# garg02/mpi-sppy

Hardware: AMD Instinct MI355X
Metric: PH scenario-iterations/sec (farmer 100k) + time to conv<1e-4 (higher is better)
Workload: dtype f64; 1 GPU; farmer crops_multiplier=1, 100000 scenarios (BASELINE configs[2]); scenarios=100000, scenarios_per_gpu=100000, n=12, m=7, nonants=3, parallelism=scenario-sharded x1, RCCL allreduce

## Files before the change

mpi-sppy_amd/csrc/phx_jit.h:

```cpp
#pragma once
#include <stdint.h>
#include <math.h>
#include <stdio.h>
#include <algorithm>
#include <sstream>
#include <string>
#include <vector>
#include "phx_setup.h"

namespace phx {

struct LaneStructure {
    int n = 0, m = 0, nnz = 0, npairs = 0, nvar = 0, nslot = 0;
    bool c_vary = false, bnd_vary = false, rhs_vary = false;
    bool scaled = false;
    std::vector<int32_t> row, col, kvar, col_slot;
    std::vector<int32_t> pair_a, pair_b, pair_pos;
    std::vector<uint8_t> lnz;
    std::vector<uint8_t> rfirst, cfirst, rempty, cempty;
    std::vector<uint8_t> lfin, ufin, fixed, blfin, bufin, eq;
    std::vector<double> Ac, dc, dr, c, lb, ub, bl, bu;
    double ipm_xs = 1.0, ipm_zs = 1.0, ipm_ws = 1.0;
    double multi_theta = 0.0;
    int multi_rounds = 0;
// ... 137 lines not shown
    o << "}; return a[k]; }\n";
}

inline void emit_dtable(std::ostringstream& o, const char* name, const std::vector<double>& v) {
    o << "  __host__ __device__ static constexpr double " << name << "(int k) { constexpr double a[] = {";
    char buf[64];
    for (size_t i = 0; i < v.size(); ++i) {
        snprintf(buf, sizeof(buf), "%a", std::isfinite(v[i]) ? v[i] : 0.0);
        o << (i ? "," : "") << buf;
    }
    if (v.empty()) o << "0.0";
    o << "}; return a[k]; }\n";
}

enum LaneKernel {
    LK_COLD, LK_COLD_AS, LK_WARM, LK_WARM_LIST, LK_MAP, LK_TAIL, LK_SEED, LK_WARM_FZ1, LK_WARM_FZR2, LK_ALL,
    LK_LIST_ALL, LK_ALL_RL, LK_ALL_PK, LK_COUNT
};
constexpr const char* LANE_KERNEL_NAMES[] = {
    "phx_lane_cold", "phx_lane_cold_as", "phx_lane_warm", "phx_lane_warm_list", "phx_lane_map", "phx_fz_tail",
    "phx_lane_seed", "phx_lane_warm_fz1", "phx_lane_warm_fzr2", "phx_lane_all", "phx_lane_list_all",
    "phx_lane_all_rl", "phx_lane_all_pk"};
static_assert(sizeof(LANE_KERNEL_NAMES) / sizeof(LANE_KERNEL_NAMES[0]) == LK_COUNT, "one name per LaneKernel");

inline std::string lane_kernel_source(const LaneStructure& L, int warm_waves = 1, bool with_map = false,
                                      int cold_waves = 1) {
    const std::string wl = with_map ? "phx_lane::warm_lane<PT, true>" : "phx_lane::warm_lane<PT, false>";
    std::ostringstream o;
    o << "#include \"phx_lane.h\"\n";
    o << "struct PT {\n";
    o << "  static constexpr int NMAX_N = " << L.n << ", NMAX_M = " << L.m << ", NMAX_K = " << L.nnz
      << ", NMAX_V = " << std::max(L.nvar, 1) << ", NMAX_S = " << std::max(L.nslot, 1) << ";\n";
    o << "  __host__ __device__ static constexpr int nvar() { return " << L.nvar << "; }\n";
    o << "  __host__ __device__ static constexpr bool scaled() { return " << (L.scaled ? "true" : "false") << "; }\n";
    o << "  __host__ __device__ static constexpr int nslot() { return " << L.nslot << "; }\n";
    o << "  __host__ __device__ static constexpr int n() { return " << L.n << "; }\n";
    o << "  __host__ __device__ static constexpr int m() { return " << L.m << "; }\n";
    o << "  __host__ __device__ static constexpr int nnz() { return " << L.nnz << "; }\n";
    o << "  __host__ __device__ static constexpr int npairs() { return " << L.npairs << "; }\n";
    o << "  __host__ __device__ static constexpr bool c_vary() { return " << (L.c_vary ? "true" : "false") << "; }\n";
    o << "  __host__ __device__ static constexpr bool bnd_vary() { return " << (L.bnd_vary ? "true" : "false")
      << "; }\n";
    o << "  __host__ __device__ static constexpr bool rhs_vary() { return " << (L.rhs_vary ? "true" : "false")
      << "; }\n";
    {
        char buf[512];
// ... 50 lines not shown
    emit_dtable(o, "bls", L.bl);
    emit_dtable(o, "bus", L.bu);
    o << "};\n";
    o << "extern \"C\" __global__ void __launch_bounds__(64, " << warm_waves
      << ") phx_lane_warm(phx_lane::LaneIO io) {\n"
         "  phx_lane::lane_stamp(io, 0);\n"
         "  if (phx_lane::gated(io.gate)) return;\n"
         "  phx_lane::zero_next_counts(io.counts_next);\n"
         "  phx_lane::lane_stamp(io, 1);\n"
         "  const int t = blockIdx.x * 64 + threadIdx.x;\n"
         "  bool still = false;\n"
         "  if (t < io.S) {\n"
         "    phx_lane::lane_stamp(io, 2);\n"
         "    still = " + wl + "(io, t);\n"
         "  }\n"
         "  phx_lane::lane_stamp(io, 3);\n"
         "  phx_lane::compact_lane(still, t, io.lanes_out, io.count_out);\n"
         "  phx_lane::lane_stamp(io, 4);\n"
         "  phx_lane::lane_stamp(io, 5);\n"
         "}\n";
    o << "extern \"C\" __global__ void __launch_bounds__(64, 1) phx_lane_warm_fz1(phx_lane::LaneIO io) {\n"
         "  phx_lane::warm_fused<PT>(io);\n"
         "}\n";
    o << "extern \"C\" __global__ void __launch_bounds__(64, 2) phx_lane_warm_fzr2(phx_lane::LaneIO io) {\n"
         "  phx_lane::warm_fused<PT, PHX_FZR2_CARRY_DEF, PHX_FZR2_PARK_DEF>(io);\n"
         "}\n";
    o << "extern \"C\" __global__ void __launch_bounds__(64, 1) phx_lane_all(phx_lane::LaneIO io, int rescue) {\n"
         "  if (phx_lane::gated(io.gate)) return;\n"
         "  phx_lane::zero_next_counts(io.counts_next);\n"
         "  const int t = blockIdx.x * 64 + threadIdx.x;\n"
         "  bool still = false;\n"
         "  if (t < io.S) still = phx_lane::all_lane<PT>(io, t, rescue);\n"
         "  phx_lane::compact_lane(still, t, io.lanes_out, io.count_out);\n"
         "}\n";
    o << "extern \"C\" __global__ void __launch_bounds__(64, 1) phx_lane_all_rl(phx_lane::LaneIO io, int rescue) {\n"
         "  if (phx_lane::gated(io.gate)) return;\n"
         "  phx_lane::zero_next_counts(io.counts_next);\n"
         "  const int t = blockIdx.x * 64 + threadIdx.x;\n"
         "  bool still = false;\n"
         "  if (t < io.S) still = phx_lane::all_lane<PT, false>(io, t, rescue);\n"
         "  phx_lane::compact_lane(still, t, io.lanes_out, io.count_out);\n"
         "}\n";
    o << "extern \"C\" __global__ void __launch_bounds__(64, 1) phx_lane_all_pk(phx_lane::LaneIO io, int rescue) {\n"
         "  __shared__ double pk[phx_lane::Data<PT>::PARK * 64];\n"
         "  if (phx_lane::gated(io.gate)) return;\n"
         "  phx_lane::zero_next_counts(io.counts_next);\n"
         "  const int t = blockIdx.x * 64 + threadIdx.x;\n"
         "  bool still = false;\n"
         "  if (t < io.S) still = phx_lane::all_lane<PT, false, true>(io, t, rescue, pk);\n"
         "  phx_lane::compact_lane(still, t, io.lanes_out, io.count_out);\n"
         "}\n";
    o << "extern \"C\" __global__ void __launch_bounds__(64) phx_fz_tail(phx_lane::LaneIO io, phx_lane::TailCopy tc) {\n"
         "  phx_lane::tail_copy(tc);\n"
         "  if (phx_lane::gated(io.gate)) return;\n"
         "  (void)phx_lane::fz_decide(io.fz, io.fz.iter);\n"
         "}\n";
    o << "extern \"C\" __global__ void __launch_bounds__(64, 4) phx_lane_map(phx_lane::LaneIO io) {\n"
         "  if (phx_lane::gated(io.gate)) return;\n"
         "  phx_lane::zero_next_counts(io.counts_next);\n"
         "  const int t = blockIdx.x * 64 + threadIdx.x;\n"
         "  bool still = false;\n"
         "  if (t < io.S) still = phx_lane::map_lane<PT>(io, t);\n"
         "  phx_lane::compact_lane(still, t, io.lanes_out, io.count_out);\n"
         "}\n";
    const std::string wlr = with_map ? "phx_lane::warm_lane<PT, true, true>" : "phx_lane::warm_lane<PT, false, true>";
    o << "#ifdef PHX_LIST_RELOAD\n#define PHX_LIST_WAVES " << warm_waves << "\n#define PHX_LIST_FN " << wl
      << "\n#else\n#define PHX_LIST_WAVES 1\n#define PHX_LIST_FN " << wlr << "\n#endif\n";
    o << "extern \"C\" __global__ void __launch_bounds__(64, PHX_LIST_WAVES"
      << ") phx_lane_warm_list(phx_lane::LaneIO io, const int* lanes, const int* count) {\n"
         "  if (phx_lane::gated(io.gate)) return;\n"
         "  const int nl = *count;\n"
         "  for (int base = blockIdx.x * 64; base < nl; base += gridDim.x * 64) {\n"
         "    const int t = base + threadIdx.x;\n"
// ... 55 lines not shown
```

mpi-sppy_amd/csrc/phx_kernels.hip:

```cpp
#include <hip/hip_runtime.h>
#include <stdio.h>
#include <string.h>
#include <math.h>
#include <string>
#include <vector>
#include <algorithm>
#include "../../include/phx.h"
#include "phx_core.h"
#include "phx_setup.h"
#include "phx_wg.h"
#include "phx_sp.h"
#include "phx_jit.h"
#include "phx_lane.h"
#include <hip/hiprtc.h>
#include <rccl/rccl.h>
#include <map>
#include <memory>
#include <mutex>
#include <stdlib.h>
#include <atomic>
#include <chrono>

#include "phx_lane_src.inc"

// ... 1698 lines not shown
    double* lane_zero_d = nullptr;
    int32_t* lane_zero_i = nullptr;
    double* lane_ipm_x = nullptr;
    double* lane_ipm_y = nullptr;
    hipFunction_t lane_warm_fn = nullptr;
    hipFunction_t lane_warm_list_fn = nullptr;
    hipFunction_t lane_map_fn = nullptr;
    hipFunction_t lane_tail_fn = nullptr;
    hipFunction_t lane_seed_fn = nullptr;
    hipFunction_t lane_warm_fz1_fn = nullptr;
    hipFunction_t lane_warm_fzr2_fn = nullptr;
    hipFunction_t lane_all_fn = nullptr;
    hipFunction_t lane_list_all_fn = nullptr;
    uint32_t* aset = nullptr;
    double* lane_map = nullptr;
    uint64_t* lane_stamps = nullptr;
    const double *lane_Av = nullptr, *lane_lb = nullptr, *lane_ub = nullptr, *lane_bl = nullptr,
                 *lane_bu = nullptr;
    bool have_aset = false;
    bool aset_fresh = false;
    std::unique_ptr<LaneStructure> lane_L;
    int lane_ww = 2, lane_cw = 1;
    std::string lane_defs;
    LaneMod mod_ph, mod_fix;
    bool fix_built = false;
    bool fix_ok = false;
    bool fix_lane = false;
    double *fix_lb = nullptr, *fix_ub = nullptr;
    bool ovr_base_ok = false;
    const double* fix_vals = nullptr;
    const int32_t* fix_idx = nullptr;
    int32_t* donor_dev = nullptr;
    int donor_cap = 0;
    std::vector<int32_t> donor_lo, donor_hi;
    const void* donor_key[3] = {nullptr, nullptr, nullptr};
    int donor_key_n[2] = {0, 0};
    const double *ph_W = nullptr, *ph_rho = nullptr, *ph_xbar = nullptr;
    const int32_t* ph_idx = nullptr;
    int32_t ph_W_on = 0, ph_prox_on = 0;
    bool ph_dirty = false;
    int32_t* counts = nullptr;
    unsigned int* tickets = nullptr;
    int32_t* lane_counts = nullptr;
    int lane_parity = 0;
    std::string jit_info = "off: not built";
    int32_t* flags_dummy = nullptr;
// ... 570 lines not shown
            const char* mapenv = getenv("PHX_LANE_MAP");
            const bool want_map = mw <= 512 && mapenv && atoi(mapenv) == 1;
            const char* cw = getenv("PHX_COLD_WAVES");
            std::string src = lane_kernel_source(L, ww ? std::max(1, atoi(ww)) : 2, want_map,
                                                 cw ? std::max(1, atoi(cw)) : 1);
            if (const char* defs = getenv("PHX_LANE_DEFS")) {
                std::string pre, tok;
                for (const char* p = defs;; ++p) {
                    if (*p == ' ' || *p == 0) {
                        const size_t eq = tok.find('=');
                        if (eq != std::string::npos) tok[eq] = ' ';
                        if (!tok.empty()) pre += "#define " + tok + "\n";
                        tok.clear();
                        if (*p == 0) break;
                    } else {
                        tok += *p;
                    }
                }
                src = pre + src;
                ctx->lane_defs = pre;
            }
            ctx->lane_ww = ww ? std::max(1, atoi(ww)) : 2;
            ctx->lane_cw = cw ? std::max(1, atoi(cw)) : 1;
            if (const char* dump = getenv("PHX_LANE_SRC_DUMP")) {
                if (FILE* f = fopen(dump, "w")) {
                    fputs(src.c_str(), f);
                    fclose(f);
                }
            }
            LaneFns fns{};
            const std::string err = jit_compile(src, &fns);
            if (!err.empty()) fns = LaneFns{};
            ctx->lane_cold_fn = fns.fn[phx::LK_COLD];
            ctx->lane_cold_as_fn = fns.fn[phx::LK_COLD_AS];
            ctx->lane_warm_fn = fns.fn[phx::LK_WARM];
            ctx->lane_warm_list_fn = fns.fn[phx::LK_WARM_LIST];
            ctx->lane_map_fn = fns.fn[phx::LK_MAP];
            ctx->lane_tail_fn = fns.fn[phx::LK_TAIL];
            ctx->lane_seed_fn = fns.fn[phx::LK_SEED];
            ctx->lane_warm_fz1_fn = fns.fn[phx::LK_WARM_FZ1];
            ctx->lane_warm_fzr2_fn = fns.fn[phx::LK_WARM_FZR2];
            ctx->lane_list_all_fn = fns.fn[phx::LK_LIST_ALL];
            ctx->lane_all_fn = fns.fn[phx::LK_ALL];
            bool all_rl = false, all_pk = false;
            if (err.empty()) {
                int scratch = 0;
// ... 14 lines not shown
            if (err.empty()) {
                ctx->lane_L.reset(new LaneStructure(L));
                const size_t nw = (size_t)phx_lane::aset_words(n, m) * S;
                ctx->aset = ctx->alloc<uint32_t>(nw);
                ctx->lane_ipm_x = ctx->alloc<double>((size_t)n * S);
                ctx->lane_ipm_y = ctx->alloc<double>((size_t)std::max(m, 1) * S);
                PHX_REQUIRE(ctx, ctx->lane_ipm_x != nullptr && ctx->lane_ipm_y != nullptr,
                            "phx_set_problem: out of device memory (ipm point)");
                {
                    const size_t NS = (size_t)std::max(ctx->N, 1) * S;
                    ctx->lane_zero_d = ctx->alloc<double>(NS);
                    ctx->lane_zero_i = ctx->alloc<int32_t>(NS);
                    PHX_REQUIRE(ctx, ctx->lane_zero_d != nullptr && ctx->lane_zero_i != nullptr,
                                "phx_set_problem: out of device memory (lane stand-ins)");
                    PHX_CHECK(ctx, hipMemset(ctx->lane_zero_d, 0, sizeof(double) * NS));
                    PHX_CHECK(ctx, hipMemset(ctx->lane_zero_i, 0, sizeof(int32_t) * NS));
                }
                ctx->seed_buf = ctx->alloc<int32_t>(2 * SEED_T + 2);
                ctx->seed_aset = ctx->alloc<uint32_t>((size_t)SEED_T * phx_lane::aset_words(n, m));
                PHX_REQUIRE(ctx, ctx->aset != nullptr && ctx->seed_buf != nullptr,
                            "phx_set_problem: out of device memory (aset)");
                PHX_CHECK(ctx, hipMemset(ctx->aset, 0, sizeof(uint32_t) * nw));
                if (getenv("PHX_LANE_STAMPS") && atoi(getenv("PHX_LANE_STAMPS")) == 1) {
                    const size_t ns = (size_t)nblk(S, PHX_BLOCK) * 8;
                    ctx->lane_stamps = ctx->alloc<uint64_t>(ns);
                    if (ctx->lane_stamps) PHX_CHECK(ctx, hipMemset(ctx->lane_stamps, 0, sizeof(uint64_t) * ns));
                }
                if (want_map) {
                    ctx->lane_map = ctx->alloc<double>(mw * S);
                    PHX_REQUIRE(ctx, ctx->lane_map != nullptr, "phx_set_problem: out of device memory (map)");
                }
            }
        } else {
            ctx->jit_info = "off: " + why;
        }
    }
    hipLaunchKernelGGL(k_norm_init, dim3(nblk(S, PHX_BLOCK)), dim3(PHX_BLOCK), 0, 0, St, S);
    if (launch_begin(ctx, 0, 0, nullptr)) return 1;
    PHX_CHECK(ctx, hipGetLastError());
    PHX_CHECK(ctx, hipDeviceSynchronize());
    if (ctx->wg_ok && !ctx->lane_cold_fn && getenv("PHX_WG_NO_FACTOR_CACHE") == nullptr) {
        const int64_t stride = (int64_t)m * (m | 1) + m;
        const int64_t kst = ((int64_t)n + m + 7) / 8 * 8;
        if ((double)S * (double)(stride * 8 + kst + 8 * (N + 1) + 4) <= 4e9) {
            ctx->wg.fac = ctx->alloc<double>((size_t)S * stride);
            ctx->wg.key = ctx->alloc<int8_t>((size_t)S * kst);
            ctx->wg.pkey = ctx->alloc<double>((size_t)S * (N + 1));
// ... 617 lines not shown
        lmax = std::max(lmax, (double)(s[5] - s[0]));
        ++nw;
    }
    if (!nw) return;
    {
        double lt[9] = {0}, sv[9] = {0}, lmx[9] = {0};
        int cnt[9] = {0};
        for (unsigned b = 0; b < G; ++b) {
            const uint64_t* s = h.data() + (size_t)b * 8;
            if (!s[0] || !s[5] || s[5] < s[0]) continue;
            const int r = (int)std::min<uint64_t>(s[6], 8);
            lt[r] += (double)(s[5] - s[0]);
            sv[r] += (double)(s[3] - s[2]);
            lmx[r] = std::max(lmx[r], (double)(s[5] - s[0]));
            ++cnt[r];
        }
        fprintf(stderr, "[lane stamps] by most rounds in the wave:");
        for (int r = 0; r <= 8; ++r)
            if (cnt[r])
                fprintf(stderr, " %d: %d waves, life %.2f (max %.2f) solve %.2f us;", r, cnt[r], lt[r] / cnt[r] * 0.01,
                        lmx[r] * 0.01, sv[r] / cnt[r] * 0.01);
        fprintf(stderr, "\n");
    }
    fprintf(stderr,
            "[lane stamps] waves %d span %.2f us, last start +%.2f us, first end +%.2f us; per wave lifetime "
            "%.2f us (max %.2f): prologue %.2f, update_w %.2f, solve %.2f, compact %.2f, epilogue %.2f us\n",
            nw, (tend - t0) * 0.01, (last_start - t0) * 0.01, (first_end - t0) * 0.01, life / nw * 0.01, lmax * 0.01,
            ph[0] / nw * 0.01, ph[1] / nw * 0.01, ph[2] / nw * 0.01, ph[3] / nw * 0.01, ph[4] / nw * 0.01);
    (void)hipMemset(ctx->lane_stamps, 0, sizeof(uint64_t) * h.size());
}

static int rescue_rounds(const phx_solve_opts* o) {
    return o->rescue_rounds > 0 ? o->rescue_rounds : std::max(16, 8 * std::max(1, o->as_rounds));
}

static int launch_cold(phx_ctx* ctx, phx_lane::LaneIO& io, const int32_t* lanes, const int32_t* count, unsigned grid,
                       hipStream_t st) {
    void* cargs[] = {&io, &lanes, &count};
    PHX_CHECK(ctx, hipModuleLaunchKernel(ctx->lane_cold_fn, grid, 1, 1, PHX_BLOCK, 1, 1, 0, st, cargs, nullptr));
    PHX_CHECK(ctx, hipModuleLaunchKernel(ctx->lane_cold_as_fn, grid, 1, 1, PHX_BLOCK, 1, 1, 0, st, cargs, nullptr));
    return 0;
}

static int enqueue_seeded_solve(phx_ctx* ctx, const phx_solve_opts* o, hipStream_t st, int32_t* C, double* x_out,
                                double* y_out, double* obj_out, int32_t* status_out, int32_t* iters_out,
                                int* npass_out) {
// ... 22 lines not shown
    }
    int32_t* next = ctx->lane_counts + 16 * ctx->lane_parity;
    io.warm_rounds = o->as_rounds;
    io.single_after = 1;
    io.lanes_out = ctx->lanesA;
    io.count_out = C;
    io.counts_next = next;
    {
        void* wargs[] = {&io};
        PHX_CHECK(ctx, hipModuleLaunchKernel(ctx->lane_warm_fn, G, 1, 1, PHX_BLOCK, 1, 1, 0, st, wargs, nullptr));
    }
    PHX_CHECK(ctx, hipGetLastError());
    io.counts_next = nullptr;
    io.lanes_out = ctx->lanesB;
    io.count_out = C + 1;
    io.as_rounds = std::max(io.as_rounds, rescue_rounds(o));
    const int32_t* in_l = ctx->lanesA;
    const int32_t* in_c = C;
    if (launch_cold(ctx, io, in_l, in_c, Gl, st)) return 1;
    *npass_out = 1;
    return 0;
}

static hipFunction_t fused_kernel(const phx_ctx* ctx, unsigned G) {
    static const bool fzr2_off = getenv("PHX_FZR2") && atoi(getenv("PHX_FZR2")) == 0;
    return (!fzr2_off && (int64_t)G > (int64_t)ctx->simds) ? ctx->lane_warm_fzr2_fn : ctx->lane_warm_fz1_fn;
}

static int enqueue_lane_solve(phx_ctx* ctx, const phx_solve_opts* o, hipStream_t st, int32_t* C, double* x_out,
                              double* y_out, double* obj_out, int32_t* status_out, int32_t* iters_out,
                              const int32_t* gate, hipEvent_t ev_a, hipEvent_t ev_b, hipEvent_t ev_c,
                              int* npass_out, unsigned cold_blocks = 0,
                              const phx_lane::FusedW* fz = nullptr, int mode = 0) {
    const int S = ctx->S;
    const unsigned G = nblk(S, PHX_BLOCK);
    phx_lane::LaneIO io = lane_io(ctx, o, x_out, y_out, obj_out, status_out, iters_out, gate);
    io.fz = fz ? *fz : phx_lane::FusedW{};
    if (fz) io.xbar_node = fz->stage;
    const bool warm_as = ctx->have_aset && o->as_rounds > 0 && ctx->lane_warm_fn;
    const bool use_map = ctx->lane_map != nullptr && ctx->lane_map_fn != nullptr;
    int npass = warm_as ? (use_map ? 2 : std::max(1, std::min(o->warm_passes, 8))) : 0;
    int32_t* next = ctx->lane_counts + 16 * ctx->lane_parity;
    int32_t* L[2] = {ctx->lanesA, ctx->lanesB};
    static const bool no_all = getenv("PHX_NO_ALL") && atoi(getenv("PHX_NO_ALL")) == 1;
    if (mode == 0 && !fz && warm_as && !use_map && npass == 1 && ctx->lane_all_fn && !no_all &&
        (int64_t)G <= (int64_t)ctx->simds) {
        if (ev_a) PHX_CHECK(ctx, ev_record(ctx, ev_a, st));
        io.lanes_out = L[0]; io.count_out = C;
        io.counts_next = next;
        io.warm_rounds = o->as_rounds;
        int resc = rescue_rounds(o);
        void* aargs[] = {&io, &resc};
        PHX_CHECK(ctx, hipModuleLaunchKernel(ctx->lane_all_fn, G, 1, 1, PHX_BLOCK, 1, 1, 0, st, aargs, nullptr));
        if (ev_b) PHX_CHECK(ctx, ev_record(ctx, ev_b, st));
        *npass_out = 0;
        return 0;
    }
    const unsigned Gl = std::min<unsigned>(G, 1024u);
    const unsigned Gc = cold_blocks ? std::min<unsigned>(G, cold_blocks) : Gl;
    if (ev_a) PHX_CHECK(ctx, ev_record(ctx, ev_a, st));
    for (int k = 0; k < npass && mode != 2; ++k) {
        io.lanes_out = L[k & 1]; io.count_out = C + k;
        io.counts_next = k == 0 ? next : nullptr;
        io.warm_rounds = use_map ? (k == 0 ? 0 : o->as_rounds) : (npass > 1 ? 1 : o->as_rounds);
        if (k == 0) {
            void* wargs[] = {&io};
            hipFunction_t fn = use_map ? ctx->lane_map_fn : (fz ? fused_kernel(ctx, G) : ctx->lane_warm_fn);
            PHX_CHECK(ctx, hipModuleLaunchKernel(fn, G, 1, 1, PHX_BLOCK, 1, 1, 0, st, wargs, nullptr));
            if (ev_b) PHX_CHECK(ctx, ev_record(ctx, ev_b, st));
        } else {
            const int32_t* in_l = L[(k - 1) & 1];
            const int32_t* in_c = C + k - 1;
            void* largs[] = {&io, &in_l, &in_c};
            PHX_CHECK(ctx, hipModuleLaunchKernel(ctx->lane_warm_list_fn, Gl, 1, 1, PHX_BLOCK, 1, 1, 0, st,
                                                 largs, nullptr));
        }
    }
    if (npass == 0 && ev_b) PHX_CHECK(ctx, ev_record(ctx, ev_b, st));
    *npass_out = npass;
    if (mode == 1) return 0;

    io.fz = phx_lane::FusedW{};
    if (mode == 2) io.xbar_node = ctx->ph_xbar;
    if (warm_as && !use_map) {
        const int32_t* in_l = L[(npass - 1) & 1];
        const int32_t* in_c = C + npass - 1;
        io.lanes_out = L[npass & 1]; io.count_out = C + npass;
        io.counts_next = nullptr;
        io.warm_rounds = rescue_rounds(o);
        io.single_after = 1;
        static const bool list_all_off = getenv("PHX_LIST_ALL") && atoi(getenv("PHX_LIST_ALL")) == 0;
// ... 1307 lines not shown
```

mpi-sppy_amd/csrc/phx_lane.h:

```cpp
#pragma once
#if !defined(__HIPCC_RTC__)
#include <stdint.h>
#include <math.h>
#if defined(__HIPCC__)
#include <hip/hip_runtime.h>
#endif
#else
typedef long long int64_t;
typedef int int32_t;
typedef unsigned int uint32_t;
typedef unsigned long long uint64_t;
#endif

#if defined(__HIPCC__) || defined(__HIPCC_RTC__)
#define PHX_LD __host__ __device__ __forceinline__
#define PHX_UNROLL _Pragma("unroll")
#define PHX_NOUNROLL _Pragma("nounroll")
#else
#define PHX_LD inline
#define PHX_UNROLL
#define PHX_NOUNROLL
#endif
#ifdef PHX_IPM_PASS_ROLLED
#define PHX_IPM_PASS_LOOP PHX_NOUNROLL
// ... 116 lines not shown
    double kkt_tol;
    double reg;
    int32_t refine;
    int32_t as_rounds;
    int32_t warm_rounds;
    int32_t single_after;
    const int32_t* gate;
    double* map;
    FusedW fz;
    uint64_t* stamps;
};

struct TailCopy {
    int32_t* left_dst;
    const int32_t* left_src;
    double* seg_dst;
    const double* seg_src;
    int32_t nseg;
    double* exp_dst;
    const double* exp_src;
};

#if defined(__HIPCC__) || defined(__HIPCC_RTC__)
__device__ __forceinline__ void lane_stamp(const LaneIO& io, int k) {
    if (io.stamps && threadIdx.x == 0) io.stamps[(uint64_t)blockIdx.x * 8 + k] = wall_clock64();
}
#endif

#if (defined(__HIPCC__) || defined(__HIPCC_RTC__)) && !defined(PHX_OUT_PLAIN)
#define PHX_OUT(lv, v) __hip_atomic_store(&(lv), (v), __ATOMIC_RELAXED, __HIP_MEMORY_SCOPE_AGENT)
#else
#define PHX_OUT(lv, v) ((lv) = (v))
#endif

PHX_LD bool gated(const int32_t* gate) { return gate && *(const volatile int32_t*)gate; }

PHX_LD void opaque(double& v) {
#if defined(__HIP_DEVICE_COMPILE__) || defined(__HIPCC_RTC__)
    __asm__ volatile("" : "+v"(v));
#else
    (void)v;
#endif
}
PHX_LD int opaque_index(int v) {
#if defined(__HIP_DEVICE_COMPILE__) || defined(__HIPCC_RTC__)
    __asm__ volatile("" : "+v"(v));
#endif
    return v;
// ... 36 lines not shown
            const double xb = io.xbar_node[fzon ? t : xi[t]];
            const double r = pon ? rv[t] : 0.0;
            const double w = won ? wv[t] : 0.0;
            qn[t] = w - r * xb;
            pn[t] = r;
            kn += 0.5 * r * xb * xb;
        }
    }
    PHX_LD Data(const LaneIO& io_, int sc_, const double* av_, const double* wv, const double* rv, const double* xbv)
        : io(io_), sc(sc_) {
        PHX_UNROLL for (int v = 0; v < PT::nvar(); ++v) av[v] = av_[v];
        const bool won = io.W_on != 0, pon = io.prox_on != 0;
        kn = 0.0;
        PHX_UNROLL for (int t = 0; t < PT::nslot(); ++t) {
            const double xb = xbv[t];
            const double r = pon ? rv[t] : 0.0;
            const double w = won ? wv[t] : 0.0;
            qn[t] = w - r * xb;
            pn[t] = r;
            kn += 0.5 * r * xb * xb;
        }
    }
    static constexpr int PARK = PT::NMAX_V + 2 * PT::NMAX_S + 1;
    PHX_LD Data(const LaneIO& io_, int sc_, const double* lds, int lane) : io(io_), sc(sc_) {
        const int l = opaque_index(lane);
        PHX_UNROLL for (int v = 0; v < PT::nvar(); ++v) av[v] = lds[v * 64 + l];
        PHX_UNROLL for (int t = 0; t < PT::nslot(); ++t) {
            qn[t] = lds[(PT::NMAX_V + t) * 64 + l];
            pn[t] = lds[(PT::NMAX_V + PT::NMAX_S + t) * 64 + l];
        }
        kn = lds[(PT::NMAX_V + 2 * PT::NMAX_S) * 64 + l];
    }
    PHX_LD void park(double* lds, int lane) const {
        PHX_UNROLL for (int v = 0; v < PT::nvar(); ++v) lds[v * 64 + lane] = av[v];
        PHX_UNROLL for (int t = 0; t < PT::nslot(); ++t) {
            lds[(PT::NMAX_V + t) * 64 + lane] = qn[t];
            lds[(PT::NMAX_V + PT::NMAX_S + t) * 64 + lane] = pn[t];
        }
        lds[(PT::NMAX_V + 2 * PT::NMAX_S) * 64 + lane] = kn;
    }
    PHX_LD double A(int k) const { return PT::kvar(k) < 0 ? PT::Ac(k) : av[PT::kvar(k)]; }
    PHX_LD double dc(int j) const { return PT::scaled() ? PT::dcs(j) : 1.0; }
    PHX_LD double dr(int i) const { return PT::scaled() ? PT::drs(i) : 1.0; }
    PHX_LD double idc(int j) const { return PT::scaled() ? PT::idcs(j) : 1.0; }
    PHX_LD double idr(int i) const { return PT::scaled() ? PT::idrs(i) : 1.0; }
    PHX_LD double c(int j) const { return PT::c_vary() ? io.c[(int64_t)j * io.S + sc] : PT::cs(j); }
    PHX_LD double q(int j) const {
        return PT::col_slot(j) >= 0 ? c(j) + dc(j) * qn[PT::col_slot(j)] : c(j);
    }
    PHX_LD double p(int j) const {
        return PT::col_slot(j) >= 0 ? dc(j) * dc(j) * pn[PT::col_slot(j)] : 0.0;
    }
    PHX_LD double l(int j) const { return PT::bnd_vary() ? io.lb[(int64_t)j * io.S + sc] : PT::lbs(j); }
    PHX_LD double u(int j) const { return PT::bnd_vary() ? io.ub[(int64_t)j * io.S + sc] : PT::ubs(j); }
    PHX_LD double bl(int i) const { return PT::rhs_vary() ? io.bl[(int64_t)i * io.S + sc] : PT::bls(i); }
    PHX_LD double bu(int i) const { return PT::rhs_vary() ? io.bu[(int64_t)i * io.S + sc] : PT::bus(i); }

    PHX_LD void matvec(const double* xv, double* ax) const {
        PHX_UNROLL for (int i = 0; i < PT::m(); ++i) if (PT::rempty(i)) ax[i] = 0.0;
        PHX_UNROLL for (int k = 0; k < PT::nnz(); ++k) {
            const double v = A(k) * xv[PT::col(k)];
            ax[PT::row(k)] = PT::rfirst(k) ? v : ax[PT::row(k)] + v;
// ... 1444 lines not shown
}

__device__ bool fz_prologue(const LaneIO& io) {
    const FusedW& f = io.fz;
    if (!f.first && fz_decide(f, f.iter - 1)) return false;
    if (f.stage[2 * f.nns] > 0.5) {
        if (blockIdx.x == 0 && threadIdx.x == 0) {
            f.ctl[1] = f.iter;
            *(volatile int32_t*)f.ctl = 2;
            publish_progress(f.prog, f.iter, 2, 0.0);
        }
        return false;
    }
    if (blockIdx.x == 0)
        for (int e = threadIdx.x; e < 2 * f.nns; e += blockDim.x) f.node_sums[e] = f.stage[e];
    return true;
}

template <class PT>
__device__ void fz_fold(const LaneIO& io, double* v) {
    const FusedW& f = io.fz;
    constexpr int NS = PT::nslot() > 0 ? PT::nslot() : 1;
    constexpr int NV = 2 * NS + 1;
    PHX_UNROLL for (int e = 0; e < NV; ++e) v[e] = wave_sum(v[e]);
    const unsigned nb = gridDim.x, b = blockIdx.x, k = b % TICKET_SHARDS;
    const unsigned nk = (nb - k + TICKET_SHARDS - 1) / TICKET_SHARDS;
    const unsigned nsh = nb < TICKET_SHARDS ? nb : TICKET_SHARDS;
    double* shard_part = f.part + (int64_t)nb * NV;
    __shared__ unsigned s_state;
    if (threadIdx.x == 0) {
        PHX_UNROLL for (int e = 0; e < NV; ++e) store_wt(&f.part[(int64_t)b * NV + e], v[e]);
        asm volatile("s_waitcnt vmcnt(0)" ::: "memory");
        PHX_HANDOFF_RELEASE();
        s_state = __hip_atomic_fetch_add(f.tk + k * TICKET_STRIDE, 1u, __ATOMIC_RELAXED,
                                         __HIP_MEMORY_SCOPE_AGENT) == nk - 1u;
    }
    __syncthreads();
    if (!s_state) return;
    PHX_HANDOFF_ACQUIRE();
    PHX_UNROLL for (int e = 0; e < NV; ++e) v[e] = 0.0;
    for (unsigned i0 = threadIdx.x; i0 < nk; i0 += 4 * 64) {
        double l[4][NV];
        PHX_UNROLL for (int u = 0; u < 4; ++u) {
            const unsigned i = i0 + 64u * u;
            PHX_UNROLL for (int e = 0; e < NV; ++e)
                l[u][e] = i < nk ? load_wt(&f.part[(int64_t)(k + TICKET_SHARDS * i) * NV + e]) : 0.0;
        }
        PHX_UNROLL for (int u = 0; u < 4; ++u) PHX_UNROLL for (int e = 0; e < NV; ++e) v[e] += l[u][e];
    }
    PHX_UNROLL for (int e = 0; e < NV; ++e) v[e] = wave_sum(v[e]);
    __syncthreads();
    if (threadIdx.x == 0) {
        PHX_UNROLL for (int e = 0; e < NV; ++e) store_wt(&shard_part[k * NV + e], v[e]);
        asm volatile("s_waitcnt vmcnt(0)" ::: "memory");
        PHX_HANDOFF_RELEASE();
        const bool last = __hip_atomic_fetch_add(f.tk + TICKET_SHARDS * TICKET_STRIDE, 1u, __ATOMIC_RELAXED,
                                                 __HIP_MEMORY_SCOPE_AGENT) == nsh - 1u;
        if (last)
            for (int q = 0; q <= TICKET_SHARDS; ++q) f.tk[q * TICKET_STRIDE] = 0u;
        s_state = last ? 2u : 0u;
    }
    __syncthreads();
    if (s_state != 2u) return;
    PHX_HANDOFF_ACQUIRE();
    const int e = threadIdx.x;
    if (e < NV) {
        double a = 0.0;
        for (unsigned q = 0; q < nsh; ++q) a += load_wt(&shard_part[q * NV + e]);
        if (e < NS) f.stage[e] = a;
        else if (e < 2 * NS) f.stage[f.nns + (e - NS)] = a;
        else {
            for (int r = 0; r < f.R; ++r) f.stage[2 * f.nns + 1 + r] = r == f.g ? a : 0.0;
            f.stage[2 * f.nns] =
                (double)__hip_atomic_load(io.count_out, __ATOMIC_RELAXED, __HIP_MEMORY_SCOPE_AGENT);
        }
    }
}

template <class PT>
__device__ void seed_block(const LaneIO& io, const int32_t* tl, int T, const uint32_t* tmpl) {
    constexpr int NC = seed_coords<PT>();
    constexpr int TS = seed_templates_staged<PT>() > 0 ? seed_templates_staged<PT>() : 1;
    constexpr int NCP = NC > 0 ? NC : 1;
    __shared__ double tc[TS * NCP];
    __shared__ double irange[NCP];
    __shared__ int tok[TS];
    const int Tn = T < TS ? T : TS;
    for (int i = threadIdx.x; i < Tn * NC; i += blockDim.x) {
// ... 144 lines not shown
    }
    double v[NV];
    PHX_UNROLL for (int e = 0; e < NV; ++e) v[e] = 0.0;
#ifndef PHX_FZ_NO_LDS_KEEP
    PHX_UNROLL for (int t = 0; t < PT::nslot(); ++t) pcv[t] = fz_keep[t * 64 + threadIdx.x];
    dl = fz_keep[NS * 64 + threadIdx.x];
#endif
    if (live) {
        v[2 * NS] = dl;
        if (!still)
            PHX_UNROLL for (int t = 0; t < PT::nslot(); ++t) {
                const double w = pcv[t] * xn[t];
                v[t] += w;
                v[NS + t] += w * xn[t];
            }
    }
    lane_stamp(io, 3);
    compact_lane(still, sc, io.lanes_out, io.count_out);
    lane_stamp(io, 4);
    fz_fold<PT>(io, v);
    lane_stamp(io, 5);
}

#endif

}
```

Baseline: 3.886 billion scenario-iterations/s.

## Add packed multi-wave fused warm kernel that rebalances slow lanes across waves

Adds a warm_fused_pack kernel that runs the fused warm solve with 128- or 256-thread blocks. Lanes still needing more active-set rounds after the first round are handed off through LDS slots, so an idle wave in the block can take them over. The fold is rewritten to work per wave (readfirstlane instead of block barriers) so it stays correct with wider blocks. A host-side LDS plan picks capacities and disables parking when LDS would overflow. The packed path is only selected when PHX_FZR2_PACK is defined, and it adds LDS pressure and extra block barriers.

Result: slower. 3.841 billion scenario-iterations/s (-1.2%).

```diff
diff --git a/mpi-sppy_amd/csrc/phx_jit.h b/mpi-sppy_amd/csrc/phx_jit.h
--- a/mpi-sppy_amd/csrc/phx_jit.h
+++ b/mpi-sppy_amd/csrc/phx_jit.h
@@ -183,6 +183,49 @@
     "phx_lane_seed", "phx_lane_warm_fz1", "phx_lane_warm_fzr2", "phx_lane_all", "phx_lane_list_all",
     "phx_lane_all_rl", "phx_lane_all_pk"};
 static_assert(sizeof(LANE_KERNEL_NAMES) / sizeof(LANE_KERNEL_NAMES[0]) == LK_COUNT, "one name per LaneKernel");
+
+constexpr int FZ_PACK_BW = 256;
+constexpr int LDS_BLOCK_MAX = 64 * 1024;
+constexpr int LDS_CU = 160 * 1024;
+inline int fz_pack_cap(const LaneStructure& L, int bw) {
+    const int64_t NV = std::max(L.nvar, 1), NS = std::max(L.nslot, 1);
+    const int64_t park = NV + 2 * NS + 1, keep = NS + 1;
+    const int64_t na = 2 * (L.n <= 32 ? 1 : 2) + 2;
+    const int64_t slot = (int64_t)(L.n + L.m) * 8 + (na + 2) * 4;
+    for (int cap = bw; cap >= 64; cap -= 64) {
+        const int64_t blk = (park + keep) * bw * 8 + cap * slot + (bw / 64) * 4 + 256;
+        if (blk <= LDS_BLOCK_MAX && (512 / bw) * blk <= LDS_CU) return cap;
+    }
+    return 0;
+}
+struct LdsPlan {
+    bool fzr2_park = true, all_pk = true;
+};
+inline LdsPlan lds_plan(const LaneStructure& L) {
+    const int64_t NV = std::max(L.nvar, 1), NS = std::max(L.nslot, 1);
+    const int64_t park = NV + 2 * NS + 1, keep = NS + 1;
+    LdsPlan p;
+    p.fzr2_park = (park + keep) * 64 * 8 <= LDS_BLOCK_MAX;
+    p.all_pk = park * 64 * 8 + 40960 <= LDS_BLOCK_MAX;
+    return p;
+}
+inline bool lane_def(const std::string& defs, const std::string& name, int* value = nullptr) {
+    const std::string key = "#define " + name;
+    for (size_t at = defs.find(key); at != std::string::npos; at = defs.find(key, at + 1)) {
+        const char c = at + key.size() < defs.size() ? defs[at + key.size()] : '\n';
+        if (c != '\n' && c != ' ') continue;
+        if (value) *value = c == ' ' ? atoi(defs.c_str() + at + key.size() + 1) : 1;
+        return true;
+    }
+    return false;
+}
+inline int fzr2_block_width(const LaneStructure& L, const std::string& defs) {
+    if (!lane_def(defs, "PHX_FZR2_PACK") || lane_def(defs, "PHX_FZR2_NO_PACK") || lane_def(defs, "PHX_FZR2_NO_PARK"))
+        return 64;
+    int bw = FZ_PACK_BW;
+    if (lane_def(defs, "PHX_FZ_PACK_BW", &bw) && bw != 128) bw = FZ_PACK_BW;
+    return fz_pack_cap(L, bw) > 0 ? bw : 64;
+}
 
 inline std::string lane_kernel_source(const LaneStructure& L, int warm_waves = 1, bool with_map = false,
                                       int cold_waves = 1) {
@@ -279,9 +322,30 @@
     o << "extern \"C\" __global__ void __launch_bounds__(64, 1) phx_lane_warm_fz1(phx_lane::LaneIO io) {\n"
          "  phx_lane::warm_fused<PT>(io);\n"
          "}\n";
-    o << "extern \"C\" __global__ void __launch_bounds__(64, 2) phx_lane_warm_fzr2(phx_lane::LaneIO io) {\n"
-         "  phx_lane::warm_fused<PT, PHX_FZR2_CARRY_DEF, PHX_FZR2_PARK_DEF>(io);\n"
-         "}\n";
+    const LdsPlan lp = lds_plan(L);
+    o << "#define PHX_FZ_CAP_FIT_256 " << fz_pack_cap(L, 256) << "\n#define PHX_FZ_CAP_FIT_128 "
+      << fz_pack_cap(L, 128) << "\n";
+    o << "#if defined(PHX_FZ_PACK_BW) && PHX_FZ_PACK_BW == 128\n"
+         "#define PHX_FZ_BW 128\n#define PHX_FZ_CAP_FIT PHX_FZ_CAP_FIT_128\n"
+         "#else\n"
+         "#define PHX_FZ_BW " << FZ_PACK_BW << "\n#define PHX_FZ_CAP_FIT PHX_FZ_CAP_FIT_256\n"
+         "#endif\n";
+    o << "#if defined(PHX_FZR2_PACK) && PHX_FZ_CAP_FIT > 0 && !defined(PHX_FZR2_NO_PACK) && !defined(PHX_FZR2_NO_PARK)\n"
+         "#if defined(PHX_FZ_PACK_CAP) && (PHX_FZ_PACK_CAP) < PHX_FZ_CAP_FIT\n"
+         "#define PHX_FZ_CAP (PHX_FZ_PACK_CAP)\n"
+         "#else\n"
+         "#define PHX_FZ_CAP PHX_FZ_CAP_FIT\n"
+         "#endif\n"
+         "extern \"C\" __global__ void __launch_bounds__(PHX_FZ_BW, 2) phx_lane_warm_fzr2(phx_lane::LaneIO io) {\n"
+         "  phx_lane::warm_fused_pack<PT, PHX_FZR2_CARRY_DEF, PHX_FZ_BW, PHX_FZ_CAP>(io);\n"
+         "}\n"
+         "#else\n"
+         "extern \"C\" __global__ void __launch_bounds__(64, 2) phx_lane_warm_fzr2(phx_lane::LaneIO io) {\n"
+         "  phx_lane::warm_fused<PT, PHX_FZR2_CARRY_DEF, PHX_FZR2_PARK_DEF && "
+      << (lp.fzr2_park ? "true" : "false")
+      << ">(io);\n"
+         "}\n"
+         "#endif\n";
     o << "extern \"C\" __global__ void __launch_bounds__(64, 1) phx_lane_all(phx_lane::LaneIO io, int rescue) {\n"
          "  if (phx_lane::gated(io.gate)) return;\n"
          "  phx_lane::zero_next_counts(io.counts_next);\n"
@@ -299,13 +363,14 @@
          "  phx_lane::compact_lane(still, t, io.lanes_out, io.count_out);\n"
          "}\n";
     o << "extern \"C\" __global__ void __launch_bounds__(64, 1) phx_lane_all_pk(phx_lane::LaneIO io, int rescue) {\n"
-         "  __shared__ double pk[phx_lane::Data<PT>::PARK * 64];\n"
-         "  if (phx_lane::gated(io.gate)) return;\n"
+      << (lp.all_pk ? "  __shared__ double pk[phx_lane::Data<PT>::PARK * 64];\n" : "")
+      << "  if (phx_lane::gated(io.gate)) return;\n"
          "  phx_lane::zero_next_counts(io.counts_next);\n"
          "  const int t = blockIdx.x * 64 + threadIdx.x;\n"
          "  bool still = false;\n"
-         "  if (t < io.S) still = phx_lane::all_lane<PT, false, true>(io, t, rescue, pk);\n"
-         "  phx_lane::compact_lane(still, t, io.lanes_out, io.count_out);\n"
+      << (lp.all_pk ? "  if (t < io.S) still = phx_lane::all_lane<PT, false, true>(io, t, rescue, pk);\n"
+                    : "  if (t < io.S) still = phx_lane::all_lane<PT, false>(io, t, rescue);\n")
+      << "  phx_lane::compact_lane(still, t, io.lanes_out, io.count_out);\n"
          "}\n";
     o << "extern \"C\" __global__ void __launch_bounds__(64) phx_fz_tail(phx_lane::LaneIO io, phx_lane::TailCopy tc) {\n"
          "  phx_lane::tail_copy(tc);\n"
diff --git a/mpi-sppy_amd/csrc/phx_kernels.hip b/mpi-sppy_amd/csrc/phx_kernels.hip
--- a/mpi-sppy_amd/csrc/phx_kernels.hip
+++ b/mpi-sppy_amd/csrc/phx_kernels.hip
@@ -1744,6 +1744,8 @@
     std::unique_ptr<LaneStructure> lane_L;
     int lane_ww = 2, lane_cw = 1;
     std::string lane_defs;
+    int fz_bw = 64;
+    int fzr2_mode = 1;
     LaneMod mod_ph, mod_fix;
     bool fix_built = false;
     bool fix_ok = false;
@@ -2360,6 +2362,8 @@
             }
             ctx->lane_ww = ww ? std::max(1, atoi(ww)) : 2;
             ctx->lane_cw = cw ? std::max(1, atoi(cw)) : 1;
+            ctx->fz_bw = phx::fzr2_block_width(L, ctx->lane_defs);
+            if (const char* fm = getenv("PHX_FZR2")) ctx->fzr2_mode = atoi(fm) == 0 ? 0 : atoi(fm) == 2 ? 2 : 1;
             if (const char* dump = getenv("PHX_LANE_SRC_DUMP")) {
                 if (FILE* f = fopen(dump, "w")) {
                     fputs(src.c_str(), f);
@@ -2420,7 +2424,7 @@
                             "phx_set_problem: out of device memory (aset)");
                 PHX_CHECK(ctx, hipMemset(ctx->aset, 0, sizeof(uint32_t) * nw));
                 if (getenv("PHX_LANE_STAMPS") && atoi(getenv("PHX_LANE_STAMPS")) == 1) {
-                    const size_t ns = (size_t)nblk(S, PHX_BLOCK) * 8;
+                    const size_t ns = (size_t)nblk(S, 256) * 4 * 8;
                     ctx->lane_stamps = ctx->alloc<uint64_t>(ns);
                     if (ctx->lane_stamps) PHX_CHECK(ctx, hipMemset(ctx->lane_stamps, 0, sizeof(uint64_t) * ns));
                 }
@@ -3084,6 +3088,11 @@
                         lmx[r] * 0.01, sv[r] / cnt[r] * 0.01);
         fprintf(stderr, "\n");
     }
+    {
+        uint64_t over = 0;
+        for (unsigned b = 0; b < G; ++b) over += h[(size_t)b * 8 + 7];
+        fprintf(stderr, "[lane stamps] hand-off overflow lanes %llu\n", (unsigned long long)over);
+    }
     fprintf(stderr,
             "[lane stamps] waves %d span %.2f us, last start +%.2f us, first end +%.2f us; per wave lifetime "
             "%.2f us (max %.2f): prologue %.2f, update_w %.2f, solve %.2f, compact %.2f, epilogue %.2f us\n",
@@ -3152,9 +3161,10 @@
     return 0;
 }
 
-static hipFunction_t fused_kernel(const phx_ctx* ctx, unsigned G) {
-    static const bool fzr2_off = getenv("PHX_FZR2") && atoi(getenv("PHX_FZR2")) == 0;
-    return (!fzr2_off && (int64_t)G > (int64_t)ctx->simds) ? ctx->lane_warm_fzr2_fn : ctx->lane_warm_fz1_fn;
+static hipFunction_t fused_kernel(const phx_ctx* ctx, unsigned G, unsigned* bw) {
+    const bool two = ctx->fzr2_mode == 2 || (ctx->fzr2_mode == 1 && (int64_t)G > (int64_t)ctx->simds);
+    *bw = two ? (unsigned)ctx->fz_bw : (unsigned)PHX_BLOCK;
+    return two ? ctx->lane_warm_fzr2_fn : ctx->lane_warm_fz1_fn;
 }
 
 static int enqueue_lane_solve(phx_ctx* ctx, const phx_solve_opts* o, hipStream_t st, int32_t* C, double* x_out,
@@ -3195,8 +3205,9 @@
         io.warm_rounds = use_map ? (k == 0 ? 0 : o->as_rounds) : (npass > 1 ? 1 : o->as_rounds);
         if (k == 0) {
             void* wargs[] = {&io};
-            hipFunction_t fn = use_map ? ctx->lane_map_fn : (fz ? fused_kernel(ctx, G) : ctx->lane_warm_fn);
-            PHX_CHECK(ctx, hipModuleLaunchKernel(fn, G, 1, 1, PHX_BLOCK, 1, 1, 0, st, wargs, nullptr));
+            unsigned bw = PHX_BLOCK;
+            hipFunction_t fn = use_map ? ctx->lane_map_fn : (fz ? fused_kernel(ctx, G, &bw) : ctx->lane_warm_fn);
+            PHX_CHECK(ctx, hipModuleLaunchKernel(fn, nblk(S, bw), 1, 1, bw, 1, 1, 0, st, wargs, nullptr));
             if (ev_b) PHX_CHECK(ctx, ev_record(ctx, ev_b, st));
         } else {
             const int32_t* in_l = L[(k - 1) & 1];
diff --git a/mpi-sppy_amd/csrc/phx_lane.h b/mpi-sppy_amd/csrc/phx_lane.h
--- a/mpi-sppy_amd/csrc/phx_lane.h
+++ b/mpi-sppy_amd/csrc/phx_lane.h
@@ -162,8 +162,12 @@
 };
 
 #if defined(__HIPCC__) || defined(__HIPCC_RTC__)
+__device__ __forceinline__ unsigned wave_in_block() {
+    return (unsigned)__builtin_amdgcn_readfirstlane((int)(threadIdx.x >> 6));
+}
+__device__ __forceinline__ unsigned lane_unit() { return blockIdx.x * (blockDim.x >> 6) + wave_in_block(); }
 __device__ __forceinline__ void lane_stamp(const LaneIO& io, int k) {
-    if (io.stamps && threadIdx.x == 0) io.stamps[(uint64_t)blockIdx.x * 8 + k] = wall_clock64();
+    if (io.stamps && (threadIdx.x & 63) == 0) io.stamps[(uint64_t)lane_unit() * 8 + k] = wall_clock64();
 }
 #endif
 
@@ -246,22 +250,22 @@
         }
     }
     static constexpr int PARK = PT::NMAX_V + 2 * PT::NMAX_S + 1;
-    PHX_LD Data(const LaneIO& io_, int sc_, const double* lds, int lane) : io(io_), sc(sc_) {
+    PHX_LD Data(const LaneIO& io_, int sc_, const double* lds, int lane, int bw = 64) : io(io_), sc(sc_) {
         const int l = opaque_index(lane);
-        PHX_UNROLL for (int v = 0; v < PT::nvar(); ++v) av[v] = lds[v * 64 + l];
+        PHX_UNROLL for (int v = 0; v < PT::nvar(); ++v) av[v] = lds[v * bw + l];
         PHX_UNROLL for (int t = 0; t < PT::nslot(); ++t) {
-            qn[t] = lds[(PT::NMAX_V + t) * 64 + l];
-            pn[t] = lds[(PT::NMAX_V + PT::NMAX_S + t) * 64 + l];
-        }
-        kn = lds[(PT::NMAX_V + 2 * PT::NMAX_S) * 64 + l];
-    }
-    PHX_LD void park(double* lds, int lane) const {
-        PHX_UNROLL for (int v = 0; v < PT::nvar(); ++v) lds[v * 64 + lane] = av[v];
+            qn[t] = lds[(PT::NMAX_V + t) * bw + l];
+            pn[t] = lds[(PT::NMAX_V + PT::NMAX_S + t) * bw + l];
+        }
+        kn = lds[(PT::NMAX_V + 2 * PT::NMAX_S) * bw + l];
+    }
+    PHX_LD void park(double* lds, int lane, int bw = 64) const {
+        PHX_UNROLL for (int v = 0; v < PT::nvar(); ++v) lds[v * bw + lane] = av[v];
         PHX_UNROLL for (int t = 0; t < PT::nslot(); ++t) {
-            lds[(PT::NMAX_V + t) * 64 + lane] = qn[t];
-            lds[(PT::NMAX_V + PT::NMAX_S + t) * 64 + lane] = pn[t];
-        }
-        lds[(PT::NMAX_V + 2 * PT::NMAX_S) * 64 + lane] = kn;
+            lds[(PT::NMAX_V + t) * bw + lane] = qn[t];
+            lds[(PT::NMAX_V + PT::NMAX_S + t) * bw + lane] = pn[t];
+        }
+        lds[(PT::NMAX_V + 2 * PT::NMAX_S) * bw + lane] = kn;
     }
     PHX_LD double A(int k) const { return PT::kvar(k) < 0 ? PT::Ac(k) : av[PT::kvar(k)]; }
     PHX_LD double dc(int j) const { return PT::scaled() ? PT::dcs(j) : 1.0; }
@@ -1752,24 +1756,26 @@
     const FusedW& f = io.fz;
     constexpr int NS = PT::nslot() > 0 ? PT::nslot() : 1;
     constexpr int NV = 2 * NS + 1;
+    const unsigned lane = threadIdx.x & 63u;
+    const unsigned nb = ((unsigned)io.S + 63u) >> 6, b = lane_unit(), k = b % TICKET_SHARDS;
+    if (b >= nb) return;
     PHX_UNROLL for (int e = 0; e < NV; ++e) v[e] = wave_sum(v[e]);
-    const unsigned nb = gridDim.x, b = blockIdx.x, k = b % TICKET_SHARDS;
     const unsigned nk = (nb - k + TICKET_SHARDS - 1) / TICKET_SHARDS;
     const unsigned nsh = nb < TICKET_SHARDS ? nb : TICKET_SHARDS;
     double* shard_part = f.part + (int64_t)nb * NV;
-    __shared__ unsigned s_state;
-    if (threadIdx.x == 0) {
+    unsigned state = 0u;
+    if (lane == 0) {
         PHX_UNROLL for (int e = 0; e < NV; ++e) store_wt(&f.part[(int64_t)b * NV + e], v[e]);
         asm volatile("s_waitcnt vmcnt(0)" ::: "memory");
         PHX_HANDOFF_RELEASE();
-        s_state = __hip_atomic_fetch_add(f.tk + k * TICKET_STRIDE, 1u, __ATOMIC_RELAXED,
-                                         __HIP_MEMORY_SCOPE_AGENT) == nk - 1u;
-    }
-    __syncthreads();
-    if (!s_state) return;
+        state = __hip_atomic_fetch_add(f.tk + k * TICKET_STRIDE, 1u, __ATOMIC_RELAXED,
+                                       __HIP_MEMORY_SCOPE_AGENT) == nk - 1u;
+    }
+    state = (unsigned)__builtin_amdgcn_readfirstlane((int)state);
+    if (!state) return;
     PHX_HANDOFF_ACQUIRE();
     PHX_UNROLL for (int e = 0; e < NV; ++e) v[e] = 0.0;
-    for (unsigned i0 = threadIdx.x; i0 < nk; i0 += 4 * 64) {
+    for (unsigned i0 = lane; i0 < nk; i0 += 4 * 64) {
         double l[4][NV];
         PHX_UNROLL for (int u = 0; u < 4; ++u) {
             const unsigned i = i0 + 64u * u;
@@ -1779,8 +1785,8 @@
         PHX_UNROLL for (int u = 0; u < 4; ++u) PHX_UNROLL for (int e = 0; e < NV; ++e) v[e] += l[u][e];
     }
     PHX_UNROLL for (int e = 0; e < NV; ++e) v[e] = wave_sum(v[e]);
-    __syncthreads();
-    if (threadIdx.x == 0) {
+    state = 0u;
+    if (lane == 0) {
         PHX_UNROLL for (int e = 0; e < NV; ++e) store_wt(&shard_part[k * NV + e], v[e]);
         asm volatile("s_waitcnt vmcnt(0)" ::: "memory");
         PHX_HANDOFF_RELEASE();
@@ -1788,12 +1794,12 @@
                                                  __HIP_MEMORY_SCOPE_AGENT) == nsh - 1u;
         if (last)
             for (int q = 0; q <= TICKET_SHARDS; ++q) f.tk[q * TICKET_STRIDE] = 0u;
-        s_state = last ? 2u : 0u;
-    }
-    __syncthreads();
-    if (s_state != 2u) return;
+        state = last ? 1u : 0u;
+    }
+    state = (unsigned)__builtin_amdgcn_readfirstlane((int)state);
+    if (!state) return;
     PHX_HANDOFF_ACQUIRE();
-    const int e = threadIdx.x;
+    const int e = (int)lane;
     if (e < NV) {
         double a = 0.0;
         for (unsigned q = 0; q < nsh; ++q) a += load_wt(&shard_part[q * NV + e]);
@@ -1984,6 +1990,187 @@
     lane_stamp(io, 5);
 }
 
-#endif
-
-}
+template <class PT, int CAP>
+struct FzSlots {
+    static constexpr int NA = 2 * (int)(sizeof(typename ASet<PT>::CMask) / 4) + 2;
+    double xz[(PT::NMAX_N + PT::NMAX_M) * CAP];
+    uint32_t aw[NA * CAP];
+    int32_t src[CAP], sc[CAP];
+};
+
+template <class PT, bool CARRY, int BW, int CAP>
+__device__ __forceinline__ void warm_fused_pack(const LaneIO& io) {
+    static_assert(BW % 64 == 0 && BW >= 64 && BW <= 256 && (BW & (BW - 1)) == 0, "block width: 64, 128 or 256");
+    static_assert(CAP % 64 == 0 && CAP >= 64 && CAP <= BW, "slot capacity: a multiple of 64 up to the block width");
+    const FusedW& f = io.fz;
+    constexpr int NS = PT::nslot() > 0 ? PT::nslot() : 1;
+    constexpr int NV = 2 * NS + 1;
+    constexpr int NVA = PT::NMAX_V, NW = aset_words(PT::NMAX_N, PT::NMAX_M);
+    constexpr int NWV = BW / 64;
+    typedef typename ASet<PT>::CMask CM;
+    const int tid = (int)threadIdx.x, wave = (int)wave_in_block(), lane = tid & 63;
+    const int sc = blockIdx.x * BW + tid;
+    const bool live = sc < io.S;
+    const int s = live ? sc : 0;
+    const int64_t S = io.S;
+    double av[NVA], xv[NS], wv[NS], rv[NS], pcv[NS];
+    uint32_t aw[NW];
+    PHX_UNROLL for (int v = 0; v < PT::nvar(); ++v) av[v] = io.Av[(int64_t)v * S + s];
+    PHX_UNROLL for (int k = 0; k < aset_words(PT::n(), PT::m()); ++k) aw[k] = io.aset[(int64_t)k * S + s];
+    PHX_UNROLL for (int j = 0; j < PT::n(); ++j) {
+        const int t = PT::col_slot(j);
+        if (t >= 0) {
+            const int64_t o = (int64_t)t * S + s;
+            xv[t] = f.x_prev[(int64_t)j * S + s];
+            wv[t] = io.W[o];
+            rv[t] = io.rho[o];
+            pcv[t] = f.pc[o];
+        }
+    }
+    lane_stamp(io, 0);
+    if (gated(io.gate)) return;
+    if (!fz_prologue(io)) return;
+    zero_next_counts(io.counts_next);
+    lane_stamp(io, 1);
+    double xb[NS], dl = 0.0;
+    PHX_UNROLL for (int t = 0; t < PT::nslot(); ++t) {
+        xb[t] = f.stage[t];
+        const double diff = xv[t] - xb[t];
+        wv[t] = wv[t] + rv[t] * diff;
+        if (live) PHX_OUT(const_cast<double*>(io.W)[(int64_t)t * S + sc], wv[t]);
+        dl += fabs(diff);
+    }
+    lane_stamp(io, 2);
+    __shared__ double fz_keep[(NS + 1) * BW];
+    __shared__ double fz_park[Data<PT>::PARK * BW];
+    __shared__ FzSlots<PT, CAP> hs;
+    __shared__ int fz_cnt[NWV];
+    PHX_UNROLL for (int t = 0; t < PT::nslot(); ++t) fz_keep[t * BW + tid] = pcv[t];
+    fz_keep[NS * BW + tid] = dl;
+    ASet<PT> a;
+    double xp[PT::NMAX_N], z[PT::NMAX_M];
+    int c0 = 2, nr = 0;
+    if (live) {
+        aset_from_words<PT>(aw, a);
+        PHX_UNROLL for (int j = 0; j < PT::n(); ++j) xp[j] = 0.0;
+        PHX_UNROLL for (int i = 0; i < PT::m(); ++i) z[i] = 0.0;
+        const Data<PT> D0(io, sc, av, wv, rv, xb);
+        D0.park(fz_park, tid, BW);
+        if (io.warm_rounds > 0) {
+            c0 = as_round<PT, CARRY, true>(io, D0, a, xp, z, 0);
+            nr = 1;
+        }
+    }
+    const bool need = live && c0 == 1 && io.warm_rounds > 1;
+    const unsigned long long nbal = __ballot(need);
+    if (lane == 0) fz_cnt[wave] = (int)__popcll(nbal);
+    __syncthreads();
+    int base = 0;
+    PHX_UNROLL for (int q = 0; q < NWV; ++q) base += q < wave ? fz_cnt[q] : 0;
+    const int slot = base + (int)__popcll(nbal & ((1ull << opaque_index(lane)) - 1ull));
+    const bool handed = need && slot < CAP;
+    if (handed) {
+        hs.src[slot] = tid;
+        hs.sc[slot] = sc;
+        int k = 0;
+        PHX_UNROLL for (int q = 0; q < (int)(sizeof(CM) / 4); ++q) hs.aw[k++ * CAP + slot] = (uint32_t)(a.f >> (32 * q));
+        PHX_UNROLL for (int q = 0; q < (int)(sizeof(CM) / 4); ++q) hs.aw[k++ * CAP + slot] = (uint32_t)(a.u >> (32 * q));
+        hs.aw[k++ * CAP + slot] = a.r;
+        hs.aw[k++ * CAP + slot] = a.l;
+        PHX_UNROLL for (int j = 0; j < PT::n(); ++j) hs.xz[j * CAP + slot] = xp[j];
+        PHX_UNROLL for (int i = 0; i < PT::m(); ++i) hs.xz[(PT::NMAX_N + i) * CAP + slot] = z[i];
+    }
+    __syncthreads();
+    if (io.stamps) {
+        const int over = (int)__popcll(__ballot(need && !handed));
+        if (lane == 0) io.stamps[(uint64_t)lane_unit() * 8 + 7] += (uint64_t)over;
+    }
+    static_assert(Data<PT>::PARK >= NS + 1, "the park column holds the result");
+    {
+        int jt = opaque_index(tid), jsc = blockIdx.x * BW + jt, c = c0;
+        bool run = live && !handed;
+        PHX_NOUNROLL for (int job = 0;;) {
+            if (run) {
+                PHX_NOUNROLL for (int r = 1; r < io.warm_rounds && c == 1; ++r, ++nr) {
+                    const Data<PT> Dr(io, jsc, fz_park, jt, BW);
+                    c = as_round<PT, CARRY, true>(io, Dr, a, xp, z, r);
+                }
+                if (c == 2) PHX_LANE_STAT(3);
+                if (c == 0) {
+                    const Data<PT> Dw(io, jsc, fz_park, jt, BW);
+                    write_certified<PT>(io, Dw, jsc, a, xp, z, 0);
+                }
+                double xr[NS];
+                PHX_UNROLL for (int t = 0; t < NS; ++t) xr[t] = 0.0;
+                if (c != 0) {
+                    aset_store<PT>(io, jsc, a);
+                    io.status[jsc] = 0;
+                    io.flags[jsc] = 0;
+                } else {
+                    PHX_UNROLL for (int j = 0; j < PT::n(); ++j)
+                        if (PT::col_slot(j) >= 0) xr[PT::col_slot(j)] = xp[j] * (PT::scaled() ? PT::dcs(j) : 1.0);
+                }
+                const int jo = opaque_index(jt);
+                PHX_UNROLL for (int t = 0; t < NS; ++t) fz_park[t * BW + jo] = xr[t];
+                fz_park[NS * BW + jo] = c != 0 ? 1.0 : 0.0;
+            }
+            if (++job == 2) break;
+            int total = 0;
+            PHX_UNROLL for (int q = 0; q < NWV; ++q) total += fz_cnt[q];
+            const int w0 = (int)((blockIdx.x + (blockIdx.x >> 8)) & (unsigned)(NWV - 1));
+            const int fs = ((((int)wave_in_block() - w0) & (NWV - 1)) << 6) + ((int)threadIdx.x & 63);
+            run = fs < (total < CAP ? total : CAP);
+            if (run) {
+                jt = hs.src[fs];
+                jsc = hs.sc[fs];
+                c = 1;
+                int k = 0;
+                CM fw = 0, uw = 0;
+                PHX_UNROLL for (int q = 0; q < (int)(sizeof(CM) / 4); ++q) fw |= (CM)hs.aw[k++ * CAP + fs] << (32 * q);
+                PHX_UNROLL for (int q = 0; q < (int)(sizeof(CM) / 4); ++q) uw |= (CM)hs.aw[k++ * CAP + fs] << (32 * q);
+                a.f = fw;
+                a.u = uw;
+                a.r = hs.aw[k++ * CAP + fs];
+                a.l = hs.aw[k++ * CAP + fs];
+                PHX_UNROLL for (int j = 0; j < PT::n(); ++j) xp[j] = hs.xz[j * CAP + fs];
+                PHX_UNROLL for (int i = 0; i < PT::m(); ++i) z[i] = hs.xz[(PT::NMAX_N + i) * CAP + fs];
+            }
+        }
+    }
+    if (io.stamps) {
+        int wmax = 0;
+        for (int q = 1; q <= 8; ++q) wmax = __ballot(nr >= q) ? q : wmax;
+        if (lane == 0) io.stamps[(uint64_t)lane_unit() * 8 + 6] = (uint64_t)wmax;
+    }
+    __syncthreads();
+    const int to = opaque_index((int)threadIdx.x), sce = blockIdx.x * BW + to;
+    const bool livee = sce < io.S;
+    bool still = false;
+    double xn[NS];
+    if (livee) {
+        still = fz_park[NS * BW + to] != 0.0;
+        PHX_UNROLL for (int t = 0; t < NS; ++t) xn[t] = fz_park[t * BW + to];
+    }
+    double v[NV];
+    PHX_UNROLL for (int e = 0; e < NV; ++e) v[e] = 0.0;
+    PHX_UNROLL for (int t = 0; t < PT::nslot(); ++t) pcv[t] = fz_keep[t * BW + to];
+    dl = fz_keep[NS * BW + to];
+    if (livee) {
+        v[2 * NS] = dl;
+        if (!still)
+            PHX_UNROLL for (int t = 0; t < PT::nslot(); ++t) {
+                const double w = pcv[t] * xn[t];
+                v[t] += w;
+                v[NS + t] += w * xn[t];
+            }
+    }
+    lane_stamp(io, 3);
+    compact_lane(still, sce, io.lanes_out, io.count_out);
+    lane_stamp(io, 4);
+    fz_fold<PT>(io, v);
+    lane_stamp(io, 5);
+}
+
+#endif
+
+}
```
